# lmchion/PowerGridworld

Hardware: AMD Instinct MI355X
Metric: agent-env-steps/sec at batch 65536, 5-agent scenario, 1/2/4/8 MI355X (higher is better)
Workload: dtype f64; 1 GPU; C4: 5-agent coordinated buildings (building+PV+storage) + IEEE-13 power flow + voltage-violation reward; pf_convergence=opendss, batch_per_gpu=65536, global_batch=65536, episode_steps=286, parallelism=env-sharded x1 (no collective on the step path)

## Files before the change

include/pgw.h:

```cpp
#ifndef PGW_H_
#define PGW_H_

#include <stdint.h>

#ifdef __cplusplus
extern "C" {
#endif

#define PGW_ABI_VERSION 33

#define PGW_OK 0
#define PGW_ERR_ARG (-1)
#define PGW_ERR_HIP (-2)

int32_t pgw_abi_version(void);
const char* pgw_last_error(void);

#define PGW_N_STRUCT_SIZES 32
int32_t pgw_struct_sizes(int64_t* out, int32_t n);

typedef struct pgw_mat {
  double* ptr;
  int64_t s_env;
  int64_t s_dim;
// ... 417 lines not shown
int32_t pgw_feeder_build(const pgw_feeder_elem* elems, int32_t n_elems, int32_t n_nodes,
                         double* Y, double* Z, double* I_src, double* V0);
int32_t pgw_pf_reduce(int32_t n_nodes, const double* Z, const double* V0, int32_t m,
                      const int32_t* elem_p, const int32_t* elem_q, int32_t n_out,
                      const int32_t* out_nodes, double* W, double* U0, double* G,
                      double* V0_out);

#define PGW_MAX_AGENTS 8

typedef struct pgw_coord_params {
  pgw_building_params bld;
  pgw_pv_params pv;
  pgw_battery_params bat;
  double vv_lo, vv_hi, vv_penalty;
  int32_t n_agents;
  int32_t act_dim, obs_dim;
  int32_t act_bld, act_pv, act_bat;
  int32_t obs_bld, obs_pv, obs_bat;
  int32_t comp_order[3];
  int32_t n_comp;
  int32_t agent_ctrl[PGW_MAX_AGENTS];
  int32_t coordinated;
  int32_t vv_row;
} pgw_coord_params;

typedef struct pgw_coord_buffers {
  pgw_mat action; int64_t act_stride_agent;
  pgw_mat obs;    int64_t obs_stride_agent;
  double* x;
  double* soc;
  double* reward;
  double* agent_power;
  double* v_out;
  double* vv;
  int32_t* iters;
  int32_t* od_list;
  int32_t* od_count;
  int32_t od_parity, pad_;
} pgw_coord_buffers;

typedef struct pgw_coord_step_info {
  pgw_building_exo ex_t, ex_next;
  double pv_pmax;
} pgw_coord_step_info;

int32_t pgw_coord_step(const pgw_coord_params* p, const pgw_pf_params* pf,
                       const pgw_pf_tables* pft, const pgw_coord_step_info* s, int64_t n,
                       pgw_coord_buffers b, void* stream);

int32_t pgw_coord_step_rows(const pgw_coord_params* p, const pgw_pf_params* pf,
                            const pgw_pf_tables* pft, const pgw_coord_step_info* s, int64_t n,
                            pgw_coord_buffers b, void* stream, uint32_t obs_rows_held);

typedef struct pgw_coord_buffers_f32 {
  pgw_matf action; int64_t act_stride_agent;
  pgw_matf obs;    int64_t obs_stride_agent;
  float* x;
  float* soc;
  float* reward;
  float* agent_power;
  float* v_out;
  float* vv;
  int32_t* iters;
  int32_t* od_list;
  int32_t* od_count;
  int32_t od_parity, pad_;
} pgw_coord_buffers_f32;

int32_t pgw_coord_step_general(const pgw_coord_params* p, const pgw_pfg_params* pf,
                               const pgw_pfg_tables* pft, const pgw_coord_step_info* s, int64_t n,
                               pgw_coord_buffers b, void* stream);

int32_t pgw_coord_step_f32(const pgw_coord_params* p, const pgw_pf_params* pf,
                           const pgw_pf_tables* pft, const pgw_coord_step_info* s, int64_t n,
                           pgw_coord_buffers_f32 b, void* stream);

int32_t pgw_coord_step_h1(const pgw_coord_params* p, const pgw_pf_params* pf, const pgw_pf_tables* pft,
                          const pgw_pf_h1* h, const pgw_coord_step_info* s, int64_t n, pgw_coord_buffers b,
                          void* stream);
int32_t pgw_coord_step_h1_f32(const pgw_coord_params* p, const pgw_pf_params* pf, const pgw_pf_tables* pft,
                              const pgw_pf_h1* h, const pgw_coord_step_info* s, int64_t n,
                              pgw_coord_buffers_f32 b, void* stream);

int32_t pgw_coord_step_prev(const pgw_coord_params* p, const pgw_pf_params* pf, const pgw_pf_tables* pft,
                            double* U, const pgw_coord_step_info* s, int64_t n, pgw_coord_buffers b,
                            void* stream);
int32_t pgw_coord_step_prev_f32(const pgw_coord_params* p, const pgw_pf_params* pf, const pgw_pf_tables* pft,
                                double* U, const pgw_coord_step_info* s, int64_t n, pgw_coord_buffers_f32 b,
                                void* stream);

enum { PGW_MC_BUILDING = 0, PGW_MC_PV = 1, PGW_MC_STORAGE = 2, PGW_MC_EV = 3 };

typedef struct pgw_mc_component {
  int32_t kind, pad_;
  pgw_mat action;
  pgw_mat obs;
  double* real_power;
} pgw_mc_component;

typedef struct pgw_mc_step_dyn {
  pgw_building_exo bld_ex_t, bld_ex_next;
  pgw_ev_step_info ev_step;
  double pv_pmax, pad_;
} pgw_mc_step_dyn;

typedef struct pgw_mc_step_args {
// ... 240 lines not shown
```

powergridworld_amd/_lib.py:

```python
import ctypes as C
import os

import torch

_HERE = os.path.dirname(os.path.abspath(__file__))
LIB_PATH = os.environ.get("PGW_LIB_PATH") or os.path.join(_HERE, "libpgw.so")
ABI_VERSION = 33

f64, i32, i64, u64, vp = C.c_double, C.c_int32, C.c_int64, C.c_uint64, C.c_void_p
P = C.POINTER

BLD_MAX_OBS = 24
EV_MAX_WORDS = 16
MAX_COMP = 8
PF_MAX_M = 16
PF_MAX_CTRL = 8
PFG_MAX_M = 128
PFG_MAX_CHK = 256
MAX_AGENTS = 8


class PgwError(RuntimeError):
    pass

# ... 128 lines not shown
                ("x_ldc", f64), ("vbase", f64), ("incr", f64), ("min_tap", f64), ("max_tap", f64),
                ("delay", f64), ("vlimit", f64)]


class RegParams(C.Structure):
    _fields_ = [("n_reg", i32), ("r_reg", i32), ("n_phase", i32), ("n_ctrl", i32),
                ("phase", RegPhase * REG_MAX_PHASES), ("ctrl", RegCtrl * REG_MAX_CTRL), ("S", vp),
                ("rho", vp)]


PF_EXACT, PF_OPENDSS, PF_OPENDSS_STEP = 0, 1, 2


class PredMeta(C.Structure):
    _fields_ = [("tstar", f64), ("left", i32), ("right", i32)]


class FeederElem(C.Structure):
    _fields_ = [("kind", i32), ("nphases", i32), ("node1", i32 * 3), ("node2", i32 * 3),
                ("conn1", i32), ("conn2", i32), ("r", f64 * 9), ("x", f64 * 9), ("c", f64 * 9),
                ("length", f64), ("freq", f64), ("kv1", f64), ("kv2", f64), ("kva", f64),
                ("pct_r1", f64), ("pct_r2", f64), ("xhl", f64), ("tap1", f64), ("tap2", f64),
                ("basekv", f64), ("pu", f64),
                ("angle", f64), ("mvasc3", f64), ("mvasc1", f64), ("x1r1", f64), ("x0r0", f64),
                ("nwindings", i32), ("conn3", i32), ("wnode", i32 * 18), ("kv3", f64), ("kva2", f64),
                ("kva3", f64), ("pct_r3", f64), ("tap3", f64), ("xht", f64), ("xlt", f64)]


class CoordParams(C.Structure):
    _fields_ = [("bld", BuildingParams), ("pv", PVParams), ("bat", BatteryParams),
                ("vv_lo", f64), ("vv_hi", f64), ("vv_penalty", f64), ("n_agents", i32),
                ("act_dim", i32), ("obs_dim", i32), ("act_bld", i32), ("act_pv", i32),
                ("act_bat", i32), ("obs_bld", i32), ("obs_pv", i32), ("obs_bat", i32),
                ("comp_order", i32 * 3), ("n_comp", i32), ("agent_ctrl", i32 * MAX_AGENTS),
                ("coordinated", i32), ("vv_row", i32)]


class CoordBuffers(C.Structure):
    _fields_ = [("action", Mat), ("act_stride_agent", i64), ("obs", Mat), ("obs_stride_agent", i64),
                ("x", vp), ("soc", vp), ("reward", vp), ("agent_power", vp), ("v_out", vp),
                ("vv", vp), ("iters", vp), ("od_list", vp), ("od_count", vp), ("od_parity", i32),
                ("pad_", i32)]


class CoordBuffersF32(C.Structure):
    _fields_ = [("action", Matf), ("act_stride_agent", i64), ("obs", Matf), ("obs_stride_agent", i64),
                ("x", vp), ("soc", vp), ("reward", vp), ("agent_power", vp), ("v_out", vp),
                ("vv", vp), ("iters", vp), ("od_list", vp), ("od_count", vp), ("od_parity", i32),
                ("pad_", i32)]


class CoordStepInfo(C.Structure):
    _fields_ = [("ex_t", BuildingExo), ("ex_next", BuildingExo), ("pv_pmax", f64)]


HS_MAX_VEHICLES, HS_MAX_DEV = 64, 4


class MCComponent(C.Structure):
    _fields_ = [("kind", i32), ("pad_", i32), ("action", Mat), ("obs", Mat), ("real_power", vp)]


class MCStepDyn(C.Structure):
    _fields_ = [("bld_ex_t", BuildingExo), ("bld_ex_next", BuildingExo), ("ev_step", EVStepInfo),
                ("pv_pmax", f64), ("pad_", f64)]


class MCStepArgs(C.Structure):
    _fields_ = [("n_comp", i32), ("pad_", i32), ("comp", MCComponent * 4),
                ("bld", BuildingParams), ("bld_ex_t", BuildingExo), ("bld_ex_next", BuildingExo),
                ("bld_ext", BuildingExt), ("bld_x", vp), ("bld_reward_state", vp),
                ("pv", PVParams), ("pv_pmax", f64), ("pv_min_voltage", vp),
                ("bat", BatteryParams), ("bat_soc", vp),
                ("ev", EVParams), ("ev_step", EVStepInfo), ("ev_endp", vp), ("ev_req", vp),
                ("ev_charging", vp), ("ev_reward", vp), ("real_power", vp), ("reward", vp),
                ("dyn", vp), ("clock", vp), ("n_dyn", i32), ("pad2_", i32)]


class MCComponentF32(C.Structure):
    _fields_ = [("kind", i32), ("pad_", i32), ("action", Matf), ("obs", Matf), ("real_power", vp)]


class MCStepArgsF32(C.Structure):
    _fields_ = [(nm, MCComponentF32 * 4) if nm == "comp" else (nm, tp) for nm, tp in MCStepArgs._fields_]


MA_MAX_SLOTS = 8


class MAStepArgs(C.Structure):
    _fields_ = [("n_comp", i32), ("pad_", i32), ("comp", MCComponent * MA_MAX_SLOTS),
                ("bld", BuildingParams), ("bld_ex_t", BuildingExo), ("bld_ex_next", BuildingExo),
                ("bld_ext", BuildingExt), ("bld_x", vp), ("bld_reward_state", vp),
                ("pv", PVParams), ("pv_pmax", f64), ("pv_min_voltage", vp),
                ("bat", BatteryParams), ("bat_soc", vp),
                ("ev", EVParams), ("ev_step", EVStepInfo), ("ev_endp", vp), ("ev_req", vp),
                ("ev_charging", vp), ("ev_reward", vp),
                ("pv2", PVParams), ("pv2_pmax", f64), ("pv2_min_voltage", vp),
                ("slot_agent", i32 * MA_MAX_SLOTS), ("slot_pv2", i32 * MA_MAX_SLOTS),
                ("slot_reward", vp * MA_MAX_SLOTS), ("band_lo", f64), ("band_hi", f64), ("band_scale", f64),
                ("n_agents", i32), ("n_bus", i32),
                ("agent_first", i32 * MAX_AGENTS), ("agent_count", i32 * MAX_AGENTS),
                ("agent_bus", i32 * MAX_AGENTS), ("agent_sum", i32 * MAX_AGENTS),
                ("agent_real_power", vp * MAX_AGENTS), ("agent_reward", vp * MAX_AGENTS), ("bus_p", vp),
                ("n_waves", i32), ("pad2_", i32), ("wave_first", i32 * MA_MAX_SLOTS),
                ("wave_count", i32 * MA_MAX_SLOTS), ("wave_slot", i32 * MA_MAX_SLOTS)]
# ... 56 lines not shown
    "pgw_battery_reset": (i32, [P(BatteryParams), i64, vp, vp, Mat, vp]),
    "pgw_battery_step": (i32, [P(BatteryParams), i64, Mat, vp, Mat, vp, vp]),
    "pgw_battery_reset_f32": (i32, [P(BatteryParams), i64, vp, vp, Matf, vp]),
    "pgw_battery_step_f32": (i32, [P(BatteryParams), i64, Matf, vp, Matf, vp, vp]),
    "pgw_pv_obs": (i32, [P(PVParams), i64, f64, vp, Mat, vp]),
    "pgw_pv_step": (i32, [P(PVParams), i64, f64, Mat, vp, Mat, vp, vp]),
    "pgw_building_reset": (i32, [P(BuildingParams), P(BuildingExo), i64, vp, vp, vp, BuildingExt,
                                 Mat, vp]),
    "pgw_building_step": (i32, [P(BuildingParams), P(BuildingExo), P(BuildingExo), i64, Mat, vp, vp,
                                vp, vp, i32, BuildingExt, Mat, vp]),
    "pgw_ev_reset": (i32, [P(EVParams), i64, vp, vp, vp, vp]),
    "pgw_ev_reset_tables": (i32, [P(EVParams), i64, vp, vp, vp, vp]),
    "pgw_pv_obs_f32": (i32, [P(PVParams), i64, f64, vp, Matf, vp]),
    "pgw_pv_step_f32": (i32, [P(PVParams), i64, f64, Matf, vp, Matf, vp, vp]),
    "pgw_building_reset_f32": (i32, [P(BuildingParams), P(BuildingExo), i64, vp, vp, vp, BuildingExt, Matf, vp]),
    "pgw_building_step_f32": (i32, [P(BuildingParams), P(BuildingExo), P(BuildingExo), i64, Matf, vp, vp, vp, vp,
                                    i32, BuildingExt, Matf, vp]),
    "pgw_ev_reset_f32": (i32, [P(EVParams), i64, vp, vp, vp, vp]),
    "pgw_ev_reset_tables_f32": (i32, [P(EVParams), i64, vp, vp, vp, vp]),
    "pgw_ev_step_f32": (i32, [P(EVParams), P(EVStepInfo), i64, Matf, vp, vp, vp, Matf, vp, vp, vp]),
    "pgw_ev_step": (i32, [P(EVParams), P(EVStepInfo), i64, Mat, vp, vp, vp, Mat, vp, vp, vp]),
    "pgw_ev_step_lanes": (i32, [P(EVParams), P(EVStepInfo), i64, Mat, vp, vp, vp, Mat, vp, vp, vp]),
    "pgw_ev_row": (i32, [i32]),
    "pgw_agent_reduce": (i32, [P(ReduceArgs), i64, vp, vp, vp]),
    "pgw_pf_solve": (i32, [P(PFParams), P(PFTables), i64, vp, vp, vp, vp, vp]),
    "pgw_pf_solve_f32": (i32, [P(PFParams), P(PFTables), i64, vp, vp, vp, vp, vp]),
    "pgw_pf_solve_h1": (i32, [P(PFParams), P(PFTables), P(PFH1), i64, vp, vp, vp, vp, vp]),
    "pgw_pf_solve_h1_f32": (i32, [P(PFParams), P(PFTables), P(PFH1), i64, vp, vp, vp, vp, vp]),
    "pgw_pf_prev_reset": (i32, [P(PFParams), P(PFTables), vp, i64, vp]),
    "pgw_pf_solve_prev": (i32, [P(PFParams), P(PFTables), vp, i64, vp, vp, vp, vp, vp]),
    "pgw_pf_solve_prev_f32": (i32, [P(PFParams), P(PFTables), vp, i64, vp, vp, vp, vp, vp]),
    "pgw_pf_solve_general": (i32, [P(PFGParams), P(PFGTables), i64, vp, vp, vp, vp, vp]),
    "pgw_reg_factor": (i32, [P(RegParams), i64, vp, vp, vp, vp]),
    "pgw_reg_control": (i32, [P(RegParams), i64, vp, vp, vp, vp, vp, vp]),
    "pgw_pf_solve_regulated": (i32, [P(PFGParams), P(PFGTables), P(RegParams), i64, vp, vp, vp, vp, i32, vp, vp,
                                     vp, vp]),
    "pgw_pf_padded_m": (i32, [i32]),
    "pgw_voltage_band_penalty": (i32, [i64, vp, f64, f64, f64, vp, vp]),
    "pgw_pf_pack_size": (i64, [i32]),
    "pgw_timing_start": (i32, [i32]),
    "pgw_debug_pf_trace": (i32, [vp]),
    "pgw_debug_mc_trace": (i32, [vp]),
    "pgw_pf_pred_meta": (i32, [P(PFParams), i32, i32, vp, vp, vp, vp]),
    "pgw_pf_pred_pack": (i32, [P(PFParams), i32, i32, vp, vp, vp]),
    "pgw_timing_stop": (i32, [vp, vp]),
    "pgw_stream_copy": (i32, [vp, vp, i64, i32, P(C.c_float), vp]),
    "pgw_pf_pack": (i32, [P(PFParams), vp, vp, vp, vp, vp]),
    "pgw_feeder_build": (i32, [P(FeederElem), i32, i32, vp, vp, vp, vp]),
    "pgw_pf_reduce": (i32, [i32, vp, vp, i32, vp, vp, i32, vp, vp, vp, vp, vp]),
    "pgw_coord_step": (i32, [P(CoordParams), P(PFParams), P(PFTables), P(CoordStepInfo), i64,
                             CoordBuffers, vp]),
    "pgw_coord_step_rows": (i32, [P(CoordParams), P(PFParams), P(PFTables), P(CoordStepInfo), i64,
                                  CoordBuffers, vp, C.c_uint32]),
    "pgw_coord_step_f32": (i32, [P(CoordParams), P(PFParams), P(PFTables), P(CoordStepInfo), i64,
                                 CoordBuffersF32, vp]),
    "pgw_coord_step_general": (i32, [P(CoordParams), P(PFGParams), P(PFGTables), P(CoordStepInfo), i64,
                                     CoordBuffers, vp]),
    "pgw_coord_step_h1": (i32, [P(CoordParams), P(PFParams), P(PFTables), P(PFH1), P(CoordStepInfo), i64,
                                CoordBuffers, vp]),
    "pgw_coord_step_h1_f32": (i32, [P(CoordParams), P(PFParams), P(PFTables), P(PFH1), P(CoordStepInfo), i64,
                                    CoordBuffersF32, vp]),
    "pgw_coord_step_prev": (i32, [P(CoordParams), P(PFParams), P(PFTables), vp, P(CoordStepInfo), i64,
                                  CoordBuffers, vp]),
    "pgw_coord_step_prev_f32": (i32, [P(CoordParams), P(PFParams), P(PFTables), vp, P(CoordStepInfo), i64,
                                      CoordBuffersF32, vp]),
    "pgw_hs_reset": (i32, [P(HSParams), P(HSStepInfo), i64, vp, HSBuffers, vp]),
    "pgw_mc_agent_step": (i32, [P(MCStepArgs), i64, vp]),
    "pgw_mc_agent_step_f32": (i32, [P(MCStepArgsF32), i64, vp]),
    "pgw_mc_ev_split_mode": (i32, [i32, P(i32)]),
    "pgw_graph_begin": (i32, [vp]),
    "pgw_graph_end": (i32, [vp, P(vp)]),
    "pgw_graph_launch": (i32, [vp, vp]),
    "pgw_graph_destroy": (i32, [vp]),
    "pgw_hs_step": (i32, [P(HSParams), P(HSStepInfo), i64, HSBuffers, vp]),
    "pgw_hs_reset_f32": (i32, [P(HSParams), P(HSStepInfo), i64, vp, HSBuffersF32, vp]),
    "pgw_hs_step_f32": (i32, [P(HSParams), P(HSStepInfo), i64, HSBuffersF32, vp]),
    "pgw_ma_step": (i32, [P(MAStepArgs), P(PFParams), P(PFTables), i64, vp, vp, vp]),
    "pgw_ma_step_f32": (i32, [P(MAStepArgsF32), P(PFParams), P(PFTables), i64, vp, vp, vp]),
}

EXPORTED = sorted(_SIGS)

STRUCTS = [Mat, BatteryParams, PVParams, BuildingParams, BuildingExo, BuildingExt, EVParams,
           EVStepInfo, ReduceArgs, PFParams, PFTables, FeederElem, CoordParams, CoordBuffers,
           CoordStepInfo, PredMeta, HSParams, HSStepInfo, HSBuffers, MCStepArgs, Matf, CoordBuffersF32,
           MAStepArgs, PFGElem, PFGParams, PFGTables, RegParams, MCStepDyn, PFOD, MCStepArgsF32,
           ODCertifyModel, MAStepArgsF32]

_lib = None


def lib():
    global _lib
    if _lib is not None:
        return _lib
    if not os.path.exists(LIB_PATH):
        raise PgwError("libpgw.so not found at %s -- build it with "
                       "`python -c 'import __graft_entry__ as g; g.build()'` or "
                       "`make -C powergridworld_amd/csrc`" % LIB_PATH)
    h = C.CDLL(LIB_PATH)
    for name, (res, args) in _SIGS.items():
        fn = getattr(h, name)
        fn.restype = res
        fn.argtypes = args
    if h.pgw_abi_version() != ABI_VERSION:
        raise PgwError("libpgw ABI %d != expected %d (rebuild)" % (h.pgw_abi_version(), ABI_VERSION))
# ... 86 lines not shown
```

powergridworld_amd/checkpoint.py:

```python
import datetime
import numbers
import warnings

import numpy as np
import torch

_SKIP_NAMES = ("version", "_ver", "cache", "_lib", "_memo", "keepalive", "voltages")
_SKIP_EXACT = ("history", "_hist", "_bv")
_SKIP_TABLES = ("_od_start", "_od_resp", "_od_vresp", "_od_qrec", "_pred_table", "_pred_sig", "_pred_meta",
                "_pred_grid",
                "od_list", "od_count")
_SCALARS = (bool, numbers.Number, str, type(None), datetime.datetime, datetime.date, np.generic)


def _ours(obj):
    mod = type(obj).__module__ or ""
    return mod.startswith("powergridworld_amd")


def _skip(name):
    n = str(name).lower()
    return n in _SKIP_EXACT or n in _SKIP_TABLES or any(s in n for s in _SKIP_NAMES)


def _walk(obj, path, out, seen):
    if id(obj) in seen:
        return
    seen = seen | {id(obj)}
    if isinstance(obj, dict):
        items = [(k, v) for k, v in obj.items() if isinstance(k, (str, int))]
    elif isinstance(obj, (list, tuple)):
        items = list(enumerate(obj))
    elif _ours(obj) and hasattr(obj, "__dict__"):
        items = list(vars(obj).items())
    else:
        return
    for k, v in items:
        if _skip(k):
            continue
        p = "%s.%s" % (path, k) if path else str(k)
        if isinstance(v, torch.Tensor):
            if v._base is not None:
                out.append((p + "#base", None, None, v._base))
            else:
                out.append((p, obj, k, v))
        elif isinstance(v, torch.Generator):
            out.append((p, obj, k, v))
        elif isinstance(v, np.ndarray):
            if v.size <= 1 << 16 and not isinstance(obj, (list, tuple, dict)):
                out.append((p, obj, k, v))
        elif isinstance(v, _SCALARS) and not isinstance(obj, (list, tuple, dict)):
            out.append((p, obj, k, v))
        elif isinstance(v, (dict, list, tuple)) or (_ours(v) and hasattr(v, "__dict__")):
            _walk(v, p, out, seen)


def _leaves(env):
    out = []
    _walk(env, "", out, set())
    return out

# ... 58 lines not shown
```

powergridworld_amd/csrc/pgw_pf.hip:

```cpp
#include <algorithm>
#include <cstdlib>
#include <cmath>
#include <type_traits>
#include <atomic>
#include <vector>

#include "pgw_common.h"
#include "pgw_od_certify.h"

static std::atomic<bool> g_pf_trace_on{false};

namespace pgw {

template <int B, int E, class F>
__device__ __forceinline__ void static_for(F&& f) {
  if constexpr (B < E) {
    f(std::integral_constant<int, B>{});
    static_for<B + 1, E>(f);
  }
}

template <int M> struct PFBlock {
  static constexpr int kTri = M * (M + 1) / 2;
  static constexpr int kU0re = 3 * kTri, kU0im = kU0re + M, kU0sum = kU0im + M;
// ... 791 lines not shown
    const S2 v = ld_act(reinterpret_cast<const S2*>(ap + j * b.action.s_dim));
    in[0].av[j] = (double)v.x;
    in[1].av[j] = (double)v.y;
  }
  S* xp = b.x + (int64_t)a * 5 * n + e;
#pragma unroll
  for (int z = 0; z < 5; ++z) {
    const S2 v = *reinterpret_cast<const S2*>(xp + z * n);
    in[0].xs[z] = (double)v.x;
    in[1].xs[z] = (double)v.y;
  }
  S* socp = b.soc + (int64_t)a * n + e;
  {
    const S2 v = *reinterpret_cast<const S2*>(socp);
    in[0].soc = (double)v.x;
    in[1].soc = (double)v.y;
  }
  S* op = b.obs.ptr + a * b.obs_stride_agent + e;
  std_agent_compute<2>(p, dv, s, pv_ob, in, [&](int slot, const double (&v)[2]) {
    const S2 w = {(S)v[0], (S)v[1]};
    if (slot < kSlotSoc) *reinterpret_cast<S2*>(xp + slot * n) = w;
    else if (slot == kSlotSoc) *reinterpret_cast<S2*>(socp) = w;
    else if (slot < kSlotPower)
      __builtin_nontemporal_store(w, reinterpret_cast<S2*>(op + (slot - kSlotObs) * b.obs.s_dim));
    else if (slot == kSlotPower) *reinterpret_cast<S2*>(b.agent_power + (int64_t)a * n + e) = w;
    else *reinterpret_cast<S2*>(b.reward + (int64_t)a * n + e) = w;
  });
}

template <class Bufs>
static bool pairs_ok(const Bufs& b, int64_t n) {
  using S = std::remove_pointer_t<decltype(b.soc)>;
  const auto al = [](const void* q) { return (reinterpret_cast<uintptr_t>(q) & (2 * sizeof(S) - 1)) == 0; };
  return n % 2 == 0 && b.action.s_env == 1 && b.obs.s_env == 1 && b.action.s_dim % 2 == 0 &&
         b.obs.s_dim % 2 == 0 && b.act_stride_agent % 2 == 0 && b.obs_stride_agent % 2 == 0 &&
         al(b.action.ptr) && al(b.obs.ptr) && al(b.x) && al(b.soc) && al(b.agent_power) &&
         al(b.reward);
}

static bool coord_is_std(const pgw_coord_params& p) {
  static const int sel[5][4] = {{0, 7, 6, 1}, {0, 7, 6, 1}, {0, 7, 5, 1}, {0, 7, 5, 1}, {0, 7, 5, 1}};
  static const int nbr[5][4] = {{1, 2, 3, 4}, {0, 2, 3, 4}, {0, 1, 3, 4}, {0, 1, 2, 4}, {0, 1, 2, 3}};
  if (p.n_comp != 3 || p.comp_order[0] != 0 || p.comp_order[1] != 1 || p.comp_order[2] != 2)
    return false;
  if (p.act_bld != 0 || p.act_pv != 6 || p.act_bat != 7 || p.act_dim != 8) return false;
  if (p.obs_bld != 0 || p.obs_pv != 15 || p.obs_bat != 16 || p.obs_dim != 17) return false;
  if (p.pv.grid_aware || p.bld.n_obs != 15) return false;
  for (int z = 0; z < 5; ++z)
    for (int j = 0; j < 4; ++j)
      if (p.bld.sel[z][j] != sel[z][j] || p.bld.nbr[z][j] != nbr[z][j]) return false;
  for (int j = 0; j < 15; ++j)
    if (p.bld.obs_var[j] != 5 + j) return false;
  return true;
}

struct CoordPFArgs {
  int32_t n_agents, coordinated, vv_row;
  int32_t agent_ctrl[PGW_MAX_AGENTS];
  double vv_lo, vv_hi, vv_penalty;
};

template <int M, bool UB, bool GC, bool KEEP, class Bufs>
__global__ void __launch_bounds__(kBlock) k_coord_pf(CoordPFArgs c, PFArgs a, pgw_pf_tables t,
                                                     int64_t n, Bufs b) {
  using Sto = std::remove_pointer_t<decltype(b.reward)>;
  const int64_t e = (int64_t)blockIdx.x * kBlock + threadIdx.x;
  const bool valid = e < n;
  long long* const trace = g_pf_trace;
  double rp[PGW_MAX_AGENTS];
  const int64_t ec = valid ? e : 0;
#pragma unroll
  for (int ag = 0; ag < PGW_MAX_AGENTS; ++ag)
    rp[ag] = (double)b.agent_power[(int64_t)min(ag, c.n_agents - 1) * n + ec] *
             ((valid && ag < c.n_agents) ? 1.0 : 0.0);
  constexpr bool kKeep = KEEP || !UB || GC;
  __shared__ double s_rows[kKeep ? kRowsLds : 1];
  bool rows_lds = false;
  if constexpr (kKeep) rows_lds = pf_rows_stage<M>(t, a.n_out, s_rows);
  PFSolver<M, UB, GC> S;
  S.load(a, t.block);
  pf_trace(trace, 0);
  double cp[PGW_PF_MAX_CTRL], cq[PGW_PF_MAX_CTRL];
#pragma unroll
  for (int s = 0; s < PGW_PF_MAX_CTRL; ++s) {
    cp[s] = 0.0;
    cq[s] = 0.0;
  }
#pragma unroll
  for (int ag = 0; ag < PGW_MAX_AGENTS; ++ag) {
    const int slot = ag < c.n_agents ? c.agent_ctrl[ag] : -1;
#pragma unroll
    for (int s = 0; s < PGW_PF_MAX_CTRL; ++s) cp[s] = (s == slot) ? cp[s] + rp[ag] : cp[s];
  }
  S.powers(a, cp, cq, 1.0);
  pf_trace(trace, 1);
  S.template initial<!(KEEP || !UB || GC)>(a, t, e, valid);
  pf_trace(trace, 2);
  double v0r, v0i, ir[M], ii[M];
  const int it = S.template iterate<kKeep>(a.max_iter, valid, v0r, v0i, ir, ii);
  pf_trace(trace, 3);
  const double v0 = sqrt(fma(v0i, v0i, v0r * v0r));
  pf_trace(trace, 4);
  if constexpr (kKeep) __syncthreads();
  double vsel = v0;
  if constexpr (kKeep)
    pf_rows_out<M>(t, rows_lds, s_rows, a.n_out, ir, ii, [&](int o, double v) {
// ... 2996 lines not shown
int32_t pgw_coord_step_prev_f32(const pgw_coord_params* p, const pgw_pf_params* pf, const pgw_pf_tables* pft,
                                double* U, const pgw_coord_step_info* s, int64_t n, pgw_coord_buffers_f32 b,
                                void* stream) {
  return coord_step_prev(p, pf, pft, U, s, n, b, stream);
}

int32_t pgw_pf_solve_h1(const pgw_pf_params* p, const pgw_pf_tables* t, const pgw_pf_h1* h, int64_t n,
                        const double* ctrl_p, const double* ctrl_q, double* v_out, int32_t* iters,
                        void* stream) {
  return pf_solve_h1(p, t, h, n, ctrl_p, ctrl_q, v_out, iters, stream);
}

int32_t pgw_pf_solve_h1_f32(const pgw_pf_params* p, const pgw_pf_tables* t, const pgw_pf_h1* h, int64_t n,
                            const float* ctrl_p, const float* ctrl_q, float* v_out, int32_t* iters,
                            void* stream) {
  return pf_solve_h1(p, t, h, n, ctrl_p, ctrl_q, v_out, iters, stream);
}

int32_t pgw_coord_step_h1(const pgw_coord_params* p, const pgw_pf_params* pf, const pgw_pf_tables* pft,
                          const pgw_pf_h1* h, const pgw_coord_step_info* s, int64_t n, pgw_coord_buffers b,
                          void* stream) {
  return coord_step_h1(p, pf, pft, h, s, n, b, stream);
}

int32_t pgw_coord_step_h1_f32(const pgw_coord_params* p, const pgw_pf_params* pf, const pgw_pf_tables* pft,
                              const pgw_pf_h1* h, const pgw_coord_step_info* s, int64_t n,
                              pgw_coord_buffers_f32 b, void* stream) {
  return coord_step_h1(p, pf, pft, h, s, n, b, stream);
}

int32_t pgw_pf_solve(const pgw_pf_params* p, const pgw_pf_tables* t, int64_t n,
                     const double* ctrl_p, const double* ctrl_q, double* v_out, int32_t* iters,
                     void* stream) {
  return pf_solve(p, t, n, ctrl_p, ctrl_q, v_out, iters, stream);
}

int32_t pgw_pf_solve_f32(const pgw_pf_params* p, const pgw_pf_tables* t, int64_t n,
                         const float* ctrl_p, const float* ctrl_q, float* v_out, int32_t* iters,
                         void* stream) {
  return pf_solve(p, t, n, ctrl_p, ctrl_q, v_out, iters, stream);
}

int32_t pgw_coord_step(const pgw_coord_params* p, const pgw_pf_params* pf, const pgw_pf_tables* pft,
                       const pgw_coord_step_info* s, int64_t n, pgw_coord_buffers b, void* stream) {
  return coord_step(p, pf, pft, s, n, b, stream);
}

int32_t pgw_coord_step_rows(const pgw_coord_params* p, const pgw_pf_params* pf, const pgw_pf_tables* pft,
                            const pgw_coord_step_info* s, int64_t n, pgw_coord_buffers b, void* stream,
                            uint32_t obs_rows_held) {
  return coord_step(p, pf, pft, s, n, b, stream, obs_rows_held);
}

int32_t pgw_coord_step_f32(const pgw_coord_params* p, const pgw_pf_params* pf,
                           const pgw_pf_tables* pft, const pgw_coord_step_info* s, int64_t n,
                           pgw_coord_buffers_f32 b, void* stream) {
  return coord_step(p, pf, pft, s, n, b, stream);
}

}
```

powergridworld_amd/multiagent_env.py:

```python
from abc import abstractmethod
from collections.abc import Mapping
from typing import Dict, Tuple, Union

import ctypes as C
import itertools
import os
import struct

import numpy as np
import pandas as pd
import torch

from powergridworld_amd import _lib
from powergridworld_amd.base import (ComponentEnv, MultiComponentEnv, as_action, oob_poll, owns_fused_hooks,
                                     resolve_env_class)
from powergridworld_amd.log import logger

try:
    from ray.rllib.env.multi_agent_env import MultiAgentEnv as Env
except ImportError:
    Env = object
    logger.warning("rllib MultiAgentEnv not found, using generic object class")

_KIND_ID = {"building": 0, "pv": 1, "storage": 2}

OBS_ROWS_UNIFORM = (10, 11, 12, 14, 15)
_OBS_ROWS_ALL = sum(1 << j for j in OBS_ROWS_UNIFORM)
_POPCOUNT = {m: bin(m).count("1") for m in
             (sum(1 << j for j, on in zip(OBS_ROWS_UNIFORM, bits) if on)
              for bits in itertools.product((0, 1), repeat=len(OBS_ROWS_UNIFORM)))}


def obs_rows_key(comfort_lb, comfort_ub, T_oa, time_of_day, pv_pmax):
    return struct.unpack("<5q", struct.pack("<5d", comfort_lb, comfort_ub, T_oa, time_of_day, pv_pmax))


def obs_rows_held(held_key, key):
    if held_key is None:
        return 0
    if held_key == key:
        return _OBS_ROWS_ALL
    mask = 0
    for j, a, b in zip(OBS_ROWS_UNIFORM, held_key, key):
        if a == b:
            mask |= 1 << j
    return mask


def resolve_pf_class(cls):
    from powergridworld_amd.distribution_system.opendss import OpenDSSSolver
    from powergridworld_amd.distribution_system.powerflow import PowerFlowSolver
    if isinstance(cls, type) and issubclass(cls, PowerFlowSolver):
        return cls
    if getattr(cls, "__name__", None) == "OpenDSSSolver":
        return OpenDSSSolver
    raise TypeError("unsupported power flow solver class %r" % (cls,))


class MultiAgentEnv(Env):

    fused_reward_transform = None

    def __init__(self, common_config: dict = {}, pf_config: dict = {}, agents: list = None,
                 max_episode_steps: int = None, rescale_spaces: bool = True, num_envs: int = 1,
                 device=None, fused: Union[bool, str] = "auto", record_history: bool = False,
                 dtype=None, history_capacity: int = None, obs_row_skip: bool = True, **kwargs):
        self.common_config = common_config
        self._obs_rows = {"on": bool(obs_row_skip) and os.environ.get("PGW_OBS_ROW_SKIP", "1") != "0",
                          "skipped": 0, "key": None}
        self.rescale_spaces = rescale_spaces
        assert len(agents) > 0, "need at least one agent!"
        self.num_envs = int(num_envs)
        self.device = _lib.require_device(device)
        self.dtype = _lib.storage_dtype(dtype)
        if self.dtype != torch.float64 and fused is False:
            raise ValueError("dtype=%s needs the fused path" % self.dtype)
        self.start_time = pd.Timestamp(common_config["start_time"])
        self.end_time = pd.Timestamp(common_config["end_time"])
        self.control_timedelta = common_config["control_timedelta"]
        self.pf_config = pf_config
        self.max_episode_steps = max_episode_steps if max_episode_steps is not None else np.inf
        self.episode_step = None
        self.time = None
        self.history = None
        self.voltages = None
        self.obs_dict = {}
        self.record_history = record_history
        self._times, self._end_step = [], 10 ** 12
        self._time_at(0)

        self.oob_count = torch.zeros(1, dtype=torch.int64, device=self.device)
        self._make_agents(agents, torch.float64)
        self.agent_name_bus_map = {a["name"]: a["bus"] for a in agents}
        self.agent_names = list(set([a.name for a in self.agents]))
        assert len(self.agent_names) == len(agents), "all agents need unique names"

        pf_cls = resolve_pf_class(pf_config["cls"])
        self.pf_solver = pf_cls(**pf_config["config"], num_envs=self.num_envs, device=self.device)

        self.observation_space = {agent.name: agent.observation_space for agent in self.agents}
        self.action_space = {agent.name: agent.action_space for agent in self.agents}

        self._fused = None
        self._ma = None
        self._fused_steps = 0
        self._at_reset = False
        self._q_zero = all(type(a).reactive_power is ComponentEnv.reactive_power for a in self.agents)
        if fused:
            why = self._fusable()
            if why is None and self.dtype != torch.float64:
                why = self._f32_fusable()
                if why is not None:
                    raise ValueError("dtype=%s: %s" % (self.dtype, why))
            if why is None:
                self._setup_fused()
            else:
                if self.dtype != torch.float64:
                    try:
                        self._make_agents(agents, self.dtype)
                    except NotImplementedError as err:
                        raise ValueError("dtype=%s: %s" % (self.dtype, err))
                why_ma = self._ma_fusable()
# ... 29 lines not shown
                            **_config, **self.common_config)
            new_agent._bind_oob(self.oob_count)
            self.agents.append(new_agent)

    @abstractmethod
    def get_external_obs_vars(self, agent: Union[ComponentEnv, MultiComponentEnv]) -> dict:
        kwargs = {}
        if "bus_voltage" in agent.obs_labels:
            kwargs["bus_voltage"] = self.pf_solver.get_bus_voltage_by_name(
                self.agent_name_bus_map[agent.name])
        if "max_voltage" in agent.obs_labels or "min_voltage" in agent.obs_labels:
            solver = self.pf_solver
            if self.voltages is getattr(solver, "bus_voltages", None) and hasattr(solver, "voltage_extrema"):
                vmin, vmax = solver.voltage_extrema()
            else:
                stacked = torch.stack(list(self.voltages.values()))
                vmin, vmax = stacked.min(0).values, stacked.max(0).values
            if "max_voltage" in agent.obs_labels:
                kwargs["max_voltage"] = vmax
            if "min_voltage" in agent.obs_labels:
                kwargs["min_voltage"] = vmin
        return kwargs

    def reward_transform(self, rew_dict) -> dict:
        return rew_dict

    def meta_transform(self, meta) -> dict:
        return meta

    def _time_at(self, step):
        times = self._times
        if step >= len(times):
            n = max(2 * len(times), step + 1, 512)
            self._times = times = [self.start_time + i * self.control_timedelta for i in range(n)]
            self._end_step = next((i for i, t in enumerate(times) if t >= self.end_time), n + 10 ** 9)
        return times[step]

    @property
    def obs_row_skip(self):
        return self._obs_rows["on"]

    @obs_row_skip.setter
    def obs_row_skip(self, on):
        self._obs_rows["on"] = bool(on)
        self._obs_rows["key"] = None

    @property
    def obs_rows_skipped(self):
        return self._obs_rows["skipped"]

    def _obs_rows_forget(self):
        self._obs_rows["key"] = None

    def reset(self) -> Dict[str, any]:
        self._obs_rows_forget()
        self.episode_step = 0
        self._resets = self.__dict__.get("_resets", 0) + 1
        oob_poll(self.oob_count)
        self.time = self._time_at(0)
        self.history = {"timestamp": [], "voltage": [], "agent_power_p": []}
        if self._hist is not None:
            self._hist["t"] = 0
            self.pf_solver.bind_output(None)
            if self._fused is not None:
                for ai, agent in enumerate(self.agents):
                    agent._real_power = self._fused["agent_power"][ai]
        self.pf_solver.calculate_power_flow(current_time=self.time)
        self._at_reset = True
        self.voltages = self.pf_solver.get_bus_voltages()
        if self._fused is not None and len(self.pf_solver.output_names) < self.pf_solver.feeder.n:
            self.voltages = self.pf_solver.bus_voltages = _FusedVoltages(
                self, self.pf_solver.bus_voltages, self._fused_steps, reset=True)
        f32 = self._fused is not None and self.dtype != torch.float64
        if f32:
            self._f32_sync(up=True)
        for agent in self.agents:
            kwargs = self.get_external_obs_vars(agent)
            _ = agent.reset(**kwargs)
        if self._fused is not None:
            self._prewarm_steps()
        if f32:
            self._f32_sync(up=False)
            return self._fused["obs_dict"]
        return self.get_obs()

    def oob_actions(self) -> torch.Tensor:
        return self.oob_count

    def get_obs(self) -> Dict[str, any]:
        obs = {}
        for agent in self.agents:
            kwargs = self.get_external_obs_vars(agent)
            obs[agent.name], _ = agent.get_obs(**kwargs)
        return obs

    def step(self, action) -> Tuple[dict, dict, dict, dict]:
        self.episode_step += 1
        self.time = self._time_at(self.episode_step)
        self._at_reset = False
        self.obs_dict = {}
        if self._fused is not None:
            obs, rew, done, meta = self._step_fused(action)
        elif self._ma is not None:
            obs, rew, done, meta = self._step_ma(action)
        else:
            obs, rew, done, meta = self._step_generic(action)
        any_done = any(done.values())
        max_steps_reached = (self.episode_step == self.max_episode_steps - 1)
        time_up = self.episode_step >= self._end_step
        d = bool(any_done or max_steps_reached or time_up)
        dones = {a.name: d for a in self.agents}
        dones["__all__"] = d
        return obs, rew, dones, meta

    def _step_generic(self, action):
        obs, rew, done, meta = {}, {}, {}, {}
        load_p, load_q = {}, {}
        agent_power_p = []
        for agent in self.agents:
            name = agent.name
            kwargs = self.get_external_obs_vars(agent)
            obs[name], rew[name], done[name], meta[name] = agent.step(action=action[name], **kwargs)
            agent_power_p.append(agent.real_power)
        if self._hist is not None:
            self.pf_solver.bind_output(self._hist["v"][self._hist["t"] % self._hist["cap"]])
        q_zero = self._q_zero
        if q_zero:
            load_p = self._bus_loads()
# ... 876 lines not shown
```

Baseline: 16.71 billion agent-env-steps/s.

## Fuse per-agent component resets into a single HIP reset kernel

Adds a k_coord_reset kernel that, in one launch over all agents and environments, runs the building warm-up state updates, writes building, PV and storage observations, and zeroes power and reward state. The Python reset path now samples the truncated-normal initial SOC with batched torch ops, then calls this kernel instead of looping over agents and components with many small launches. The fused path is gated by layout and subclass checks and falls back to per-component reset otherwise. It risks small numerical or RNG-order differences from the original reset, and it only affects reset, which runs once per 286-step episode.

```diff
diff --git a/include/pgw.h b/include/pgw.h
--- a/include/pgw.h
+++ b/include/pgw.h
@@ -493,6 +493,18 @@
                             const pgw_pf_tables* pft, const pgw_coord_step_info* s, int64_t n,
                             pgw_coord_buffers b, void* stream, uint32_t obs_rows_held);
 
+typedef struct pgw_coord_reset_args {
+  const double* init;
+  int64_t init_stride_agent;
+  int32_t sampled_init, pad_;
+  double* p_consumed[PGW_MAX_AGENTS];
+  double* reward_state[PGW_MAX_AGENTS];
+  double* storage_power[PGW_MAX_AGENTS];
+} pgw_coord_reset_args;
+
+int32_t pgw_coord_reset(const pgw_coord_params* p, const pgw_building_exo* ex0, double pv_pmax0,
+                        int64_t n, pgw_coord_buffers b, const pgw_coord_reset_args* r, void* stream);
+
 typedef struct pgw_coord_buffers_f32 {
   pgw_matf action; int64_t act_stride_agent;
   pgw_matf obs;    int64_t obs_stride_agent;
diff --git a/powergridworld_amd/_lib.py b/powergridworld_amd/_lib.py
--- a/powergridworld_amd/_lib.py
+++ b/powergridworld_amd/_lib.py
@@ -204,6 +204,12 @@
 
 class CoordStepInfo(C.Structure):
     _fields_ = [("ex_t", BuildingExo), ("ex_next", BuildingExo), ("pv_pmax", f64)]
+
+
+class CoordResetArgs(C.Structure):
+    _fields_ = [("init", vp), ("init_stride_agent", i64), ("sampled_init", i32), ("pad_", i32),
+                ("p_consumed", vp * MAX_AGENTS), ("reward_state", vp * MAX_AGENTS),
+                ("storage_power", vp * MAX_AGENTS)]
 
 
 HS_MAX_VEHICLES, HS_MAX_DEV = 64, 4
@@ -366,6 +372,7 @@
                              CoordBuffers, vp]),
     "pgw_coord_step_rows": (i32, [P(CoordParams), P(PFParams), P(PFTables), P(CoordStepInfo), i64,
                                   CoordBuffers, vp, C.c_uint32]),
+    "pgw_coord_reset": (i32, [P(CoordParams), P(BuildingExo), f64, i64, CoordBuffers, P(CoordResetArgs), vp]),
     "pgw_coord_step_f32": (i32, [P(CoordParams), P(PFParams), P(PFTables), P(CoordStepInfo), i64,
                                  CoordBuffersF32, vp]),
     "pgw_coord_step_general": (i32, [P(CoordParams), P(PFGParams), P(PFGTables), P(CoordStepInfo), i64,
diff --git a/powergridworld_amd/checkpoint.py b/powergridworld_amd/checkpoint.py
--- a/powergridworld_amd/checkpoint.py
+++ b/powergridworld_amd/checkpoint.py
@@ -6,7 +6,8 @@
 import torch
 
 _SKIP_NAMES = ("version", "_ver", "cache", "_lib", "_memo", "keepalive", "voltages")
-_SKIP_EXACT = ("history", "_hist", "_bv")
+_SKIP_EXACT = ("history", "_hist", "_bv",
+               "_fused_reset")
 _SKIP_TABLES = ("_od_start", "_od_resp", "_od_vresp", "_od_qrec", "_pred_table", "_pred_sig", "_pred_meta",
                 "_pred_grid",
                 "od_list", "od_count")
diff --git a/powergridworld_amd/csrc/pgw_pf.hip b/powergridworld_amd/csrc/pgw_pf.hip
--- a/powergridworld_amd/csrc/pgw_pf.hip
+++ b/powergridworld_amd/csrc/pgw_pf.hip
@@ -867,6 +867,86 @@
   for (int j = 0; j < 15; ++j)
     if (p.bld.obs_var[j] != 5 + j) return false;
   return true;
+}
+
+static_assert(sizeof(pgw_coord_reset_args) == 24 + 3 * 8 * PGW_MAX_AGENTS,
+              "pgw_coord_reset_args: the binding's layout (it is not in pgw_struct_sizes)");
+__global__ void __launch_bounds__(kBlock) k_coord_reset(pgw_coord_params p_, pgw_building_exo ex0,
+                                                        double pmax0, int64_t n, pgw_coord_buffers b,
+                                                        pgw_coord_reset_args r, StdDerived dv) {
+  const pgw_coord_params& p = PGW_KERNARG0(pgw_coord_params);
+  const int64_t e = (int64_t)blockIdx.x * kBlock + threadIdx.x;
+  const int a = blockIdx.y;
+  if (e >= n) return;
+  double* xp = b.x + (int64_t)a * 5 * n + e;
+  double xs[5], T[5];
+#pragma unroll
+  for (int z = 0; z < 5; ++z) xs[z] = xp[z * n];
+  const double init = r.init[(int64_t)a * r.init_stride_agent + e];
+  double *pcons = nullptr, *rstate = nullptr, *bat_rp = nullptr;
+#pragma unroll
+  for (int k = 0; k < PGW_MAX_AGENTS; ++k) {
+    pcons = a == k ? r.p_consumed[k] : pcons;
+    rstate = a == k ? r.reward_state[k] : rstate;
+    bat_rp = a == k ? r.storage_power[k] : bat_rp;
+  }
+  const pgw_building_params& B = p.bld;
+#pragma unroll
+  for (int z = 0; z < 5; ++z) T[z] = B.T_init[z];
+#pragma unroll
+  for (int it = 0; it < 2; ++it) {
+#pragma unroll
+    for (int z = 0; z < 5; ++z) {
+      const int nz = z < 2 ? 4 : (z == 2 ? 3 : 2);
+      const double u0 = ex0.T_oa - T[z];
+      const double u1 = ex0.q_cool[z];
+      const double u2 = T[nz] - T[z];
+      const double u3 = ex0.q_solar[z];
+      double bu = B.B[z][0] * u0;
+      bu = bu + B.B[z][1] * u1;
+      bu = bu + B.B[z][2] * u2;
+      bu = bu + B.B[z][3] * u3;
+      xs[z] = B.A[z] * xs[z] + bu;
+    }
+#pragma unroll
+    for (int z = 0; z < 5; ++z) {
+      double yhat = B.C[z] * xs[z];
+      double yact = T[z] - B.mean[z];
+      xs[z] = xs[z] + B.K[z] * (yact - yhat);
+    }
+  }
+#pragma unroll
+  for (int z = 0; z < 5; ++z) {
+    xp[z * n] = xs[z];
+    T[z] = B.C[z] * xs[z] + B.mean[z];
+  }
+  if (pcons) pcons[e] = 0.0;
+  if (rstate) rstate[e] = building_reward(B, T, ex0.comfort_lb, ex0.comfort_ub, 0.0);
+  double* op = b.obs.ptr + a * b.obs_stride_agent + e * b.obs.s_env;
+  const double lb = ex0.comfort_lb, ub = ex0.comfort_ub;
+  auto obs_value = [&](int j) {
+    return j < 5 ? T[j] - ub : j < 10 ? lb - T[j - 5] : j == 10 ? lb
+         : j == 11 ? ub : j == 12 ? ex0.T_oa : j == 13 ? 0.0 : ex0.time_of_day;
+  };
+  if (B.rescale) {
+#pragma unroll
+    for (int j = 0; j < 15; ++j) {
+      const double c = clip_fast(obs_value(j), B.obs_low[j], B.obs_high[j]);
+      st_obs(op + j * b.obs.s_dim, exact_div(2.0 * c - dv.obs_sum[j], dv.obs_rng[j], dv.obs_rcp[j]));
+    }
+  } else {
+#pragma unroll
+    for (int j = 0; j < 15; ++j)
+      st_obs(op + j * b.obs.s_dim, clip_fast(obs_value(j), B.obs_low[j], B.obs_high[j]));
+  }
+  st_obs(op + 15 * b.obs.s_dim, pv_obs(p.pv, pmax0));
+  const double s = r.sampled_init ? init : clip(init, p.bat.soc_min, p.bat.soc_max);
+  b.soc[(int64_t)a * n + e] = s;
+  const double sc = clip_fast(s, p.bat.soc_min, p.bat.soc_max);
+  st_obs(op + 16 * b.obs.s_dim,
+         p.bat.rescale ? exact_div(2.0 * sc - dv.bat_sum, dv.bat_rng, dv.bat_rcp) : s);
+  if (bat_rp) bat_rp[e] = 0.0;
+  b.agent_power[(int64_t)a * n + e] = 0.0;
 }
 
 struct CoordPFArgs {
@@ -3969,6 +4049,25 @@
   return coord_step(p, pf, pft, s, n, b, stream, obs_rows_held);
 }
 
+int32_t pgw_coord_reset(const pgw_coord_params* p, const pgw_building_exo* ex0, double pv_pmax0,
+                        int64_t n, pgw_coord_buffers b, const pgw_coord_reset_args* r, void* stream) {
+  PGW_REQUIRE(p && ex0 && r && r->init && b.obs.ptr && b.x && b.soc && b.agent_power && n >= 0,
+              "pgw_coord_reset: null argument");
+  PGW_REQUIRE(p->n_agents >= 1 && p->n_agents <= PGW_MAX_AGENTS, "pgw_coord_reset: n_agents %d outside 1..%d",
+              p->n_agents, PGW_MAX_AGENTS);
+  PGW_REQUIRE(p->bld.n_obs >= 0 && p->bld.n_obs <= PGW_BLD_MAX_OBS, "pgw_coord_reset: bad n_obs");
+  for (int j = 0; j < p->bld.n_obs; ++j)
+    PGW_REQUIRE(p->bld.obs_var[j] < PGW_BV_BUS_VOLTAGE || p->bld.obs_var[j] > PGW_BV_P_SETPOINT,
+                "pgw_coord_reset: the building observes bus_voltage, min_voltage, max_voltage or p_setpoint");
+  PGW_REQUIRE(!p->pv.grid_aware, "pgw_coord_reset: grid-aware PV");
+  PGW_REQUIRE(coord_is_std(*p),
+              "pgw_coord_reset: needs the standard C4 agent layout (building/pv/storage at observations 0/15/16)");
+  if (n == 0) return PGW_OK;
+  hipLaunchKernelGGL(k_coord_reset, dim3(grid_for(n), p->n_agents), dim3(kBlock), 0, (hipStream_t)stream, *p,
+                     *ex0, pv_pmax0, n, b, *r, make_std_derived(*p));
+  return check_launch("k_coord_reset");
+}
+
 int32_t pgw_coord_step_f32(const pgw_coord_params* p, const pgw_pf_params* pf,
                            const pgw_pf_tables* pft, const pgw_coord_step_info* s, int64_t n,
                            pgw_coord_buffers_f32 b, void* stream) {
diff --git a/powergridworld_amd/multiagent_env.py b/powergridworld_amd/multiagent_env.py
--- a/powergridworld_amd/multiagent_env.py
+++ b/powergridworld_amd/multiagent_env.py
@@ -4,6 +4,7 @@
 
 import ctypes as C
 import itertools
+import math
 import os
 import struct
 
@@ -33,6 +34,38 @@
 
 def obs_rows_key(comfort_lb, comfort_ub, T_oa, time_of_day, pv_pmax):
     return struct.unpack("<5q", struct.pack("<5d", comfort_lb, comfort_ub, T_oa, time_of_day, pv_pmax))
+
+
+def fused_reset_why(agents):
+    from powergridworld_amd.agents.buildings import FiveZoneROMEnv
+    from powergridworld_amd.agents.energy_storage import EnergyStorageEnv
+    from powergridworld_amd.agents.pv import PVEnv
+    own = ((FiveZoneROMEnv, ("reset", "get_obs")), (PVEnv, ("reset", "get_obs")),
+           (EnergyStorageEnv, ("reset", "get_obs", "_sample_initial_storage")))
+    for a in agents:
+        if any(getattr(type(a), h, None) is not getattr(MultiComponentEnv, h) for h in ("reset", "get_obs")):
+            return "agent %s overrides reset or get_obs" % a.name
+        if len(a.envs) != 3:
+            return "agent %s is not [building, pv, storage]" % a.name
+        for e, (base, hooks) in zip(a.envs, own):
+            if not isinstance(e, base):
+                return "agent %s is not [building, pv, storage]" % a.name
+            for h in hooks:
+                if getattr(type(e), h, None) is not getattr(base, h):
+                    return "%s overrides %s" % (type(e).__name__, h)
+    b0 = agents[0].envs[2]
+    dist0 = (b0.initial_storage_mean, b0.initial_storage_std)
+    if not all(type(v) in (int, float) for v in dist0):
+        return "initial_storage_mean / _std are not plain numbers"
+    ex0 = bytes(agents[0].envs[0]._exo[0])
+    for a in agents[1:]:
+        b = a.envs[2]
+        if type(b.initial_storage_mean) is not type(dist0[0]) or type(b.initial_storage_std) is not type(dist0[1]) \
+                or (b.initial_storage_mean, b.initial_storage_std) != dist0:
+            return "storages differ in initial_storage_mean / initial_storage_std"
+        if bytes(a.envs[0]._exo[0]) != ex0:
+            return "buildings differ in their first exogenous row"
+    return None
 
 
 def obs_rows_held(held_key, key):
@@ -64,10 +97,13 @@
     def __init__(self, common_config: dict = {}, pf_config: dict = {}, agents: list = None,
                  max_episode_steps: int = None, rescale_spaces: bool = True, num_envs: int = 1,
                  device=None, fused: Union[bool, str] = "auto", record_history: bool = False,
-                 dtype=None, history_capacity: int = None, obs_row_skip: bool = True, **kwargs):
+                 dtype=None, history_capacity: int = None, obs_row_skip: bool = True,
+                 fused_reset: bool = True, **kwargs):
         self.common_config = common_config
         self._obs_rows = {"on": bool(obs_row_skip) and os.environ.get("PGW_OBS_ROW_SKIP", "1") != "0",
                           "skipped": 0, "key": None}
+        self._fused_reset = {"on": bool(fused_reset) and os.environ.get("PGW_FUSED_RESET", "1") != "0",
+                             "resets": 0, "u": None, "why": None, "checked": False}
         self.rescale_spaces = rescale_spaces
         assert len(agents) > 0, "need at least one agent!"
         self.num_envs = int(num_envs)
@@ -203,6 +239,75 @@
     def _obs_rows_forget(self):
         self._obs_rows["key"] = None
 
+    @property
+    def fused_resets(self):
+        return self._fused_reset["resets"]
+
+    def _fused_reset_ok(self):
+        R = self._fused_reset
+        if not R["checked"]:
+            R["checked"] = True
+            if self._fused is None or self.dtype != torch.float64:
+                R["why"] = "not the fp64 fused step"
+            elif self._f32_fusable() is not None or not self._std_layout(self._fused["params"]):
+                R["why"] = "not the standard C4 agent layout"
+            else:
+                R["why"] = fused_reset_why(self.agents)
+            if R["why"] is not None:
+                logger.info("MultiAgentEnv: per-component reset (%s)", R["why"])
+        return R["on"] and R["why"] is None
+
+    def _reset_fused(self):
+        F, R = self._fused, self._fused_reset
+        n, na = self.num_envs, len(self.agents)
+        step_b = F["bufs"]
+        power0 = self.agents[0]._real_power
+        for ai, agent in enumerate(self.agents):
+            bld, pv, bat = agent.envs
+            if bld.x.data_ptr() != F["x"][ai].data_ptr() or bat.soc.data_ptr() != F["soc"][ai].data_ptr() or \
+                    bld._obs.data_ptr() != F["obs"][ai].data_ptr() or \
+                    pv._obs.data_ptr() != F["obs"][ai, 15].data_ptr() or \
+                    bat._obs.data_ptr() != F["obs"][ai, 16].data_ptr() or \
+                    agent._real_power.data_ptr() != power0.data_ptr() + 8 * n * ai or \
+                    any(t.dtype != torch.float64 or not t.is_contiguous() or t.shape != (n,)
+                        for t in (agent._real_power, bld.p_consumed, bld._reward_state, bat._real_power)):
+                return False
+        U = R["u"]
+        if U is None:
+            U = R["u"] = torch.empty((na, n), dtype=torch.float64, device=self.device)
+        bat0 = self.agents[0].envs[2]
+        for ai, agent in enumerate(self.agents):
+            torch.rand(n, generator=agent.envs[2]._gen, out=U[ai])
+        lo = 0.5 * (1.0 + math.erf(-1.0 / math.sqrt(2.0)))
+        hi = 0.5 * (1.0 + math.erf(1.0 / math.sqrt(2.0)))
+        U.mul_(hi - lo).add_(lo).mul_(2.0).sub_(1.0)
+        torch.special.erfinv(U, out=U)
+        U.mul_(math.sqrt(2.0)).mul_(bat0.initial_storage_std).add_(bat0.initial_storage_mean)
+        b = _lib.CoordBuffers()
+        b.obs, b.obs_stride_agent = step_b.obs, step_b.obs_stride_agent
+        b.x, b.soc = step_b.x, step_b.soc
+        b.agent_power = power0.data_ptr()
+        r = _lib.CoordResetArgs()
+        r.init, r.init_stride_agent, r.sampled_init = U.data_ptr(), U.stride(0), 1
+        for ai, agent in enumerate(self.agents):
+            bld, pv, bat = agent.envs
+            r.p_consumed[ai] = bld.p_consumed.data_ptr()
+            r.reward_state[ai] = bld._reward_state.data_ptr()
+            r.storage_power[ai] = bat._real_power.data_ptr()
+        bld0, pv0 = self.agents[0].envs[0], self.agents[0].envs[1]
+        _lib.check(_lib.lib().pgw_coord_reset(F["params"], bld0._exo[0], float(pv0.data[0]), n, b, r,
+                                              _lib.stream_ptr(self.device)))
+        for agent in self.agents:
+            bld, pv, bat = agent.envs
+            bld.time_index, bld._prev_viol_reward = 0, None
+            pv.index = 0
+            bat.simulation_step = 0
+            bat.get_obs()
+            agent._ep_step = 0
+        oob_poll(self.oob_count)
+        R["resets"] += 1
+        return True
+
     def reset(self) -> Dict[str, any]:
         self._obs_rows_forget()
         self.episode_step = 0
@@ -225,6 +330,9 @@
         f32 = self._fused is not None and self.dtype != torch.float64
         if f32:
             self._f32_sync(up=True)
+        if self._fused_reset_ok() and self._reset_fused():
+            self._prewarm_steps()
+            return {agent.name: {e.name: e._obs for e in agent.envs} for agent in self.agents}
         for agent in self.agents:
             kwargs = self.get_external_obs_vars(agent)
             _ = agent.reset(**kwargs)
```

New measurement: 17.40 billion agent-env-steps/s (median of 6 runs). 4.1% higher.
